# AolinFeng/PMP-VVC-TIP2023

Measured on AMD Instinct MI355X. Metric: CTUs/sec (luma QT+MTT inference+post-proc), higher is better.
Workload: dtype f16x3

## Files before the change

pmp_vvc_tip2023_amd/csrc/conv_f16x3.hip:

```cpp
#include <cstdio>
#include <type_traits>

#include "pmp_kernels.h"
#include "split3.h"

namespace pmp {

template <int KH, int KW, int NTHR = 256>
struct StagePlanH {
    unsigned off[GeoH<KH, KW, 16, NTHR>::NLD];
    unsigned valid;
};

template <int KH, int KW, int NTHR = 256>
__device__ __forceinline__ void h2_plan(StagePlanH<KH, KW, NTHR> &p, size_t plane_stride, int H, int W, int ty, int tx)
{
    typedef GeoH<KH, KW, 16, NTHR> G;
    constexpr int PY = KH / 2, PX = KW / 2;
    p.valid = 0;
#pragma unroll
    for (int k = 0; k < G::NLD; ++k) {
        const int i = min((int)threadIdx.x + k * NTHR, G::PIECES - 1);
        const int sp = i / G::PLANE, j = i - sp * G::PLANE, pix = j >> 1, half = j & 1;
        const int row = pix / G::TW, col = pix - row * G::TW;
        const int gy = ty * 16 + row - PY, gx = tx * 16 + col - PX;
        const bool in = gy >= 0 && gy < H && gx >= 0 && gx < W && (int)threadIdx.x + k * NTHR < G::PIECES;
        if (in) p.valid |= 1u << k;
        const int cy = min(max(gy, 0), H - 1), cx = min(max(gx, 0), W - 1);
        p.off[k] = (unsigned)(sp * plane_stride + ((size_t)cy * W + cx) * 16 + half * 8);
    }
}

template <int KH, int KW, int NTHR = 256>
__device__ __forceinline__ void h2_stage_load(const StagePlanH<KH, KW, NTHR> &p, const unsigned short *__restrict__ grp,
                                              u32x4 (&r)[GeoH<KH, KW, 16, NTHR>::NLD], int k0 = 0, int k1 = 1 << 20)
{
#pragma unroll
    for (int k = 0; k < GeoH<KH, KW, 16, NTHR>::NLD; ++k) {
        if (k < k0 || k >= k1) continue;
        r[k] = *reinterpret_cast<const u32x4 *>(grp + p.off[k]);
    }
}

template <int KH, int KW, int NTHR = 256>
__device__ __forceinline__ void h2_stage_store(const StagePlanH<KH, KW, NTHR> &p, u32x4 *lds, const u32x4 (&r)[GeoH<KH, KW, 16, NTHR>::NLD],
                                               int k0 = 0, int k1 = 1 << 20)
{
    typedef GeoH<KH, KW, 16, NTHR> G;
#pragma unroll
    for (int k = 0; k < G::NLD; ++k) {
        if (k < k0 || k >= k1) continue;
        const int i = min((int)threadIdx.x + k * NTHR, G::PIECES);
        const u32x4 z = {0u, 0u, 0u, 0u};
        lds[i] = ((p.valid >> k) & 1u) ? r[k] : z;
    }
}

template <int KH, int KW, int NT, bool LEAN = false>
__device__ __forceinline__ void h2_accumulate(const unsigned short *__restrict__ x, size_t plane_stride,
                                              const unsigned short *__restrict__ wpk, int C, int H, int W, int n, int ty,
                                              int tx, u32x4 *lds, f32x4 (&acc)[WaveTile<NT>::RW][WaveTile<NT>::CW])
{
    constexpr int NTHR = 256;
    typedef GeoH<KH, KW, 16, NTHR> G;
    typedef WaveTile<NT> WT;
    constexpr int RW = WT::RW, CW = WT::CW;
    const int lane = threadIdx.x & 63, wave = threadIdx.x >> 6, xl = lane & 15, g = lane >> 4;
    const int rh = wave % WT::RSPLIT, ch = wave / WT::RSPLIT;
    const int CB = C >> 4;
    const size_t grp_sz = (size_t)H * W * 16;
    const unsigned short *grp0 = x + (size_t)n * CB * grp_sz;
    constexpr bool W0DB = NT == 4;
    constexpr bool W2 = W0DB && G::TAPS == 9 && !LEAN;
    u32x4 r[G::NLD];
    StagePlanH<KH, KW, NTHR> plan;
    const bool paired = (CB & 1) == 0 && (G::TAPS & 1);
    const f16x8 *wl = reinterpret_cast<const f16x8 *>(wpk) + lane + ch * CW * 64;
    const int last = paired ? (CB / 2) * G::TAPS - 1 : CB * G::NKS - 1;
    f16x8 w0[CW], w1[CW];
    f16x8 w0n[CW];
    f16x8 w1n[CW], w0nn[CW];
    h2_plan<KH, KW, NTHR>(plan, plane_stride, H, W, ty, tx);
#pragma unroll
    for (int nt = 0; nt < CW; ++nt) {
        if (W0DB) w0n[nt] = wl[(0 * NT + nt) * 64]; else w0[nt] = wl[(0 * NT + nt) * 64];
        w1[nt] = wl[(1 * NT + nt) * 64];
        if (W2) {
            const f16x8 *w2 = wl + (size_t)min(1, last) * (2 * NT * 64);
            w0nn[nt] = w2[(0 * NT + nt) * 64]; w1n[nt] = w2[(1 * NT + nt) * 64];
        }
    }
    __syncthreads();
    h2_stage_load<KH, KW, NTHR>(plan, grp0, r);
    h2_stage_store<KH, KW, NTHR>(plan, lds, r);
    __syncthreads();
    const int pb = ((rh * RW * G::TW + xl) * 2 + (g & 1)) * 16;
    int stream = 0;
    int tapsel = g >> 1;
    constexpr int O_LAST = (((G::TAPS - 1) / KW) * G::TW + (G::TAPS - 1) % KW) * 32;
    f16x8 x0[RW], x1[RW];

    auto group = [&](auto mode_tag, auto tail_tag, int cb) {
        constexpr int MODE = decltype(mode_tag)::value;
        constexpr int TAIL = decltype(tail_tag)::value;
        constexpr bool LAST = TAIL == 2;
        constexpr int NK = MODE == 0 ? G::NKS : (MODE == 1 ? (G::TAPS - 1) / 2 : (G::TAPS - 1) / 2 + 1);
        constexpr int PER = (G::NLD + (NK > 0 ? NK : 1) - 1) / (NK > 0 ? NK : 1);
        constexpr int LAG = G::TAPS > 9 ? 3 : 2;
        constexpr bool FETCH = TAIL < 2;
        u32x4 (&rl)[G::NLD] = r;
        u32x4 (&rs)[G::NLD] = r;
        constexpr bool more = !LAST;
        const unsigned short *nxt_grp = grp0 + (size_t)min(cb + 1, CB - 1) * grp_sz;
        const int bcur = cb & 1, bprev = (cb + 1) & 1;
        const char *buf = reinterpret_cast<const char *>(lds + bcur * G::BUF);
        auto xaddr = [&](int ks) -> const char * {
            const int j = MODE == 2 ? ks - 1 : ks;
            int tA = 2 * j, tB = 2 * j + 1;
            if (MODE == 0 && tB >= G::TAPS) tB = tA;
            const int oA = ((tA / KW) * G::TW + tA % KW) * 32, oB = ((tB / KW) * G::TW + tB % KW) * 32;
            return buf + (tapsel ? oB : oA) + pb;
        };
        if constexpr (LEAN) {
            constexpr int RS = 2, SUB = RW / RS;
            const char *part = reinterpret_cast<const char *>(lds + bprev * G::BUF);
            if (NK == 0 && FETCH) h2_stage_load<KH, KW, NTHR>(plan, nxt_grp, rl);
#pragma unroll
            for (int ks = 0; ks < NK; ++ks) {
                asm volatile("" : "+v"(tapsel));
                const char *px = (MODE == 2 && ks == 0) ? (g < 2 ? part : buf) + O_LAST + pb : xaddr(ks);
                ++stream;
                const f16x8 *wf = wl + (size_t)min(stream, last) * (2 * NT * 64);
                f16x8 xa[RS], xb[RS];
                auto rd_a = [&](int h) __attribute__((always_inline)) {
#pragma unroll
                    for (int m = 0; m < RS; ++m) xa[m] = *reinterpret_cast<const f16x8 *>(px + (h * RS + m) * G::TW * 32);
                };
                auto rd_b = [&](int h) __attribute__((always_inline)) {
#pragma unroll
                    for (int m = 0; m < RS; ++m) xb[m] = *reinterpret_cast<const f16x8 *>(px + G::PLANE * 16 + (h * RS + m) * G::TW * 32);
                };
#pragma unroll
                for (int h = 0; h < SUB; ++h) {
                    rd_a(h); rd_b(h);
                    __builtin_amdgcn_sched_barrier(0);
#pragma unroll
                    for (int m = 0; m < RS; ++m)
#pragma unroll
                        for (int nt = 0; nt < CW; ++nt)
                            acc[h * RS + m][nt] = __builtin_amdgcn_mfma_f32_16x16x32_f16(w1[nt], xa[m], acc[h * RS + m][nt], 0, 0, 0);
                    __builtin_amdgcn_sched_barrier(0);
                    if (h == 0) {
#pragma unroll
                        for (int nt = 0; nt < CW; ++nt) w0[nt] = w0n[nt];
#pragma unroll
                        for (int nt = 0; nt < CW; ++nt) { w1n[nt] = wf[(1 * NT + nt) * 64]; w0n[nt] = wf[(0 * NT + nt) * 64]; }
                        if (FETCH) h2_stage_load<KH, KW, NTHR>(plan, nxt_grp, rl, ks * PER, (ks + 1) * PER);
                        if (more && ks >= LAG)
                            h2_stage_store<KH, KW, NTHR>(plan, lds + ((cb + 1) & 1) * G::BUF, rs, (ks - LAG) * PER, (ks - LAG + 1) * PER);
                    } else if (h == SUB - 1) {
#pragma unroll
                        for (int nt = 0; nt < CW; ++nt) w1[nt] = w1n[nt];
                    }
                    __builtin_amdgcn_sched_barrier(0);
#pragma unroll
                    for (int m = 0; m < RS; ++m)
#pragma unroll
                        for (int nt = 0; nt < CW; ++nt)
                            acc[h * RS + m][nt] = __builtin_amdgcn_mfma_f32_16x16x32_f16(w0[nt], xa[m], acc[h * RS + m][nt], 0, 0, 0);
                    __builtin_amdgcn_sched_barrier(0);
#pragma unroll
                    for (int m = 0; m < RS; ++m)
#pragma unroll
                        for (int nt = 0; nt < CW; ++nt)
                            acc[h * RS + m][nt] = __builtin_amdgcn_mfma_f32_16x16x32_f16(w0[nt], xb[m], acc[h * RS + m][nt], 0, 0, 0);
                    __builtin_amdgcn_sched_barrier(0);
                }
                if (MODE == 2 && ks == 0) h2_lds_barrier();
            }
        } else {
            if (NK == 0) {
                if (FETCH) h2_stage_load<KH, KW, NTHR>(plan, nxt_grp, rl);
            } else if (MODE == 2) {
                if (g >= 2) {
                    const char *pl = buf + O_LAST + pb;
#pragma unroll
                    for (int m = 0; m < RW; ++m) {
                        x0[m] = *reinterpret_cast<const f16x8 *>(pl + m * G::TW * 32);
                        x1[m] = *reinterpret_cast<const f16x8 *>(pl + G::PLANE * 16 + m * G::TW * 32);
                    }
                }
            } else {
                const char *p0x = xaddr(0);
#pragma unroll
                for (int m = 0; m < RW; ++m) x0[m] = *reinterpret_cast<const f16x8 *>(p0x + m * G::TW * 32);
            }
#pragma unroll
            for (int ks = 0; ks < NK; ++ks) {
                asm volatile("" : "+v"(tapsel));
                const char *px = (MODE == 2 && ks == 0) ? buf : xaddr(ks);
                ++stream;
                if (!(MODE == 2 && ks == 0)) {
#pragma unroll
                    for (int m = 0; m < RW; ++m) x1[m] = *reinterpret_cast<const f16x8 *>(px + G::PLANE * 16 + m * G::TW * 32);
                }
                const f16x8 *wf = wl + (size_t)min(stream, last) * (2 * NT * 64);
                __builtin_amdgcn_sched_barrier(0);
#pragma unroll
                for (int m = 0; m < RW; ++m)
#pragma unroll
                    for (int nt = 0; nt < CW; ++nt) acc[m][nt] = __builtin_amdgcn_mfma_f32_16x16x32_f16(w1[nt], x0[m], acc[m][nt], 0, 0, 0);
                __builtin_amdgcn_sched_barrier(0);
                if (W2) {
                    const f16x8 *wf2 = wl + (size_t)min(stream + 1, last) * (2 * NT * 64);
#pragma unroll
                    for (int nt = 0; nt < CW; ++nt) { w1[nt] = w1n[nt]; w0[nt] = w0n[nt]; w0n[nt] = w0nn[nt]; }
#pragma unroll
                    for (int nt = 0; nt < CW; ++nt) w1n[nt] = wf2[(1 * NT + nt) * 64];
#pragma unroll
                    for (int nt = 0; nt < CW; ++nt) w0nn[nt] = wf2[(0 * NT + nt) * 64];
                } else {
#pragma unroll
                    for (int nt = 0; nt < CW; ++nt) w1[nt] = wf[(1 * NT + nt) * 64];
                    if (W0DB) {
#pragma unroll
                        for (int nt = 0; nt < CW; ++nt) w0[nt] = w0n[nt];
#pragma unroll
                        for (int nt = 0; nt < CW; ++nt) w0n[nt] = wf[(0 * NT + nt) * 64];
                    }
                }
                if (FETCH) h2_stage_load<KH, KW, NTHR>(plan, nxt_grp, rl, ks * PER, (ks + 1) * PER);
                if (more && ks >= LAG)
                    h2_stage_store<KH, KW, NTHR>(plan, lds + ((cb + 1) & 1) * G::BUF, rs, (ks - LAG) * PER, (ks - LAG + 1) * PER);
                __builtin_amdgcn_sched_barrier(0);
#pragma unroll
                for (int m = 0; m < RW; ++m)
#pragma unroll
                    for (int nt = 0; nt < CW; ++nt) acc[m][nt] = __builtin_amdgcn_mfma_f32_16x16x32_f16(w0[nt], x0[m], acc[m][nt], 0, 0, 0);
                __builtin_amdgcn_sched_barrier(0);
                if (ks + 1 < NK) {
                    const char *pn = xaddr(ks + 1);
#pragma unroll
                    for (int m = 0; m < RW; ++m) x0[m] = *reinterpret_cast<const f16x8 *>(pn + m * G::TW * 32);
                }
                __builtin_amdgcn_sched_barrier(0);
#pragma unroll
                for (int m = 0; m < RW; ++m)
#pragma unroll
                    for (int nt = 0; nt < CW; ++nt) acc[m][nt] = __builtin_amdgcn_mfma_f32_16x16x32_f16(w0[nt], x1[m], acc[m][nt], 0, 0, 0);
                __builtin_amdgcn_sched_barrier(0);
                if (!W0DB) {
#pragma unroll
                    for (int nt = 0; nt < CW; ++nt) w0[nt] = wf[(0 * NT + nt) * 64];
                }
                __builtin_amdgcn_sched_barrier(0);
            }
            if (MODE == 1 && g < 2) {
                const char *pl = buf + O_LAST + pb;
#pragma unroll
                for (int m = 0; m < RW; ++m) {
                    x0[m] = *reinterpret_cast<const f16x8 *>(pl + m * G::TW * 32);
                    x1[m] = *reinterpret_cast<const f16x8 *>(pl + G::PLANE * 16 + m * G::TW * 32);
                }
            }
        }
        if (more) h2_stage_store<KH, KW, NTHR>(plan, lds + ((cb + 1) & 1) * G::BUF, rs, NK > LAG ? (NK - LAG) * PER : 0);
        __syncthreads();
    };

    typedef std::integral_constant<int, 0> M0;
    typedef std::integral_constant<int, 1> M1;
    typedef std::integral_constant<int, 2> M2;
    typedef std::integral_constant<int, 0> T0;
    typedef std::integral_constant<int, 1> T1;
    typedef std::integral_constant<int, 2> T2;
    if (paired) {
        for (int cb = 0; cb + 2 < CB; cb += 2) {
            group(M1{}, T0{}, cb);
            group(M2{}, T0{}, cb + 1);
        }
        group(M1{}, T1{}, CB - 2);
        group(M2{}, T2{}, CB - 1);
    } else {
        for (int cb = 0; cb + 1 < CB; ++cb) group(M0{}, T0{}, cb);
        group(M0{}, T2{}, CB - 1);
    }
}

template <int NT>
__device__ __forceinline__ void h2_epilogue(const ConvX6Args &a, f32x4 (&acc)[WaveTile<NT>::RW][WaveTile<NT>::CW], int n, int ty, int tx);

template <int NT>
__device__ __forceinline__ void h2_shortcut32(const ConvX6Args &a, int n, int ty, int tx, u32x4 *lds,
                                              f32x4 (&acc)[WaveTile<NT>::RW][WaveTile<NT>::CW])
{
    typedef WaveTile<NT> WT;
    constexpr int RW = WT::RW, CW = WT::CW;
    const int tid = threadIdx.x, lane = tid & 63, wave = tid >> 6, xl = lane & 15, g = lane >> 4;
    const int rh = wave % WT::RSPLIT, ch = wave / WT::RSPLIT;
    const int W = a.W;
    const size_t grp_sz = (size_t)a.H * W * 16;
    const unsigned short *base = a.x_sc + (size_t)n * 2 * grp_sz + ((size_t)(ty * 16) * W + tx * 16) * 16;
    __syncthreads();
    u32x4 r[8];
#pragma unroll
    for (int k = 0; k < 8; ++k) {
        const int i = tid + k * 256, grp = i >> 10, plane = (i >> 9) & 1, j = i & 511, px = j >> 1, half = j & 1;
        r[k] = *reinterpret_cast<const u32x4 *>(base + plane * a.sc_stride + grp * grp_sz + ((size_t)(px >> 4) * W + (px & 15)) * 16 + half * 8);
    }
    const f16x8 *wl = reinterpret_cast<const f16x8 *>(a.w_sc) + lane + ch * CW * 64;
    f16x8 w0[CW], w1[CW];
#pragma unroll
    for (int nt = 0; nt < CW; ++nt) { w0[nt] = wl[(0 * NT + nt) * 64]; w1[nt] = wl[(1 * NT + nt) * 64]; }
#pragma unroll
    for (int k = 0; k < 8; ++k) lds[tid + k * 256] = r[k];
    __syncthreads();
    const char *px = reinterpret_cast<const char *>(lds) + (g >> 1) * 16384 + ((rh * RW * 16 + xl) * 2 + (g & 1)) * 16;
#pragma unroll
    for (int h = 0; h < RW / 2; ++h) {
        f16x8 xa[2], xb[2];
#pragma unroll
        for (int m = 0; m < 2; ++m) {
            xa[m] = *reinterpret_cast<const f16x8 *>(px + (h * 2 + m) * 16 * 32);
            xb[m] = *reinterpret_cast<const f16x8 *>(px + 8192 + (h * 2 + m) * 16 * 32);
        }
#pragma unroll
        for (int m = 0; m < 2; ++m)
#pragma unroll
            for (int nt = 0; nt < CW; ++nt) acc[h * 2 + m][nt] = __builtin_amdgcn_mfma_f32_16x16x32_f16(w1[nt], xa[m], acc[h * 2 + m][nt], 0, 0, 0);
#pragma unroll
        for (int m = 0; m < 2; ++m)
#pragma unroll
            for (int nt = 0; nt < CW; ++nt) acc[h * 2 + m][nt] = __builtin_amdgcn_mfma_f32_16x16x32_f16(w0[nt], xa[m], acc[h * 2 + m][nt], 0, 0, 0);
#pragma unroll
        for (int m = 0; m < 2; ++m)
#pragma unroll
            for (int nt = 0; nt < CW; ++nt) acc[h * 2 + m][nt] = __builtin_amdgcn_mfma_f32_16x16x32_f16(w0[nt], xb[m], acc[h * 2 + m][nt], 0, 0, 0);
    }
}

template <int KH, int KW, int NT, int SC, bool LEAN = false>
__global__ __launch_bounds__(256, NT == 4 && !LEAN ? 2 : 3) void conv_h2_kernel(ConvX6Args a)
{
    typedef GeoH<KH, KW> G;
    __shared__ u32x4 lds[2 * G::BUF];
    const int tiles_x = a.W >> 4, tiles = tiles_x * (a.H >> 4);
    int bid = blockIdx.x;
    if ((gridDim.x & 7) == 0) bid = (bid & 7) * (gridDim.x >> 3) + (bid >> 3);
    const int n = bid / tiles, t = bid - n * tiles, ty = t / tiles_x, tx = t - ty * tiles_x;
    typedef WaveTile<NT> WT;
    constexpr int RW = WT::RW, CW = WT::CW;

    f32x4 acc[RW][CW];
#pragma unroll
    for (int m = 0; m < RW; ++m)
#pragma unroll
        for (int nt = 0; nt < CW; ++nt) acc[m][nt] = (f32x4){0.f, 0.f, 0.f, 0.f};

    h2_accumulate<KH, KW, NT, LEAN>(a.x, a.x_stride, a.w, a.Cin, a.H, a.W, n, ty, tx, lds, acc);
    if (SC == 2) h2_shortcut32<NT>(a, n, ty, tx, lds, acc);
    else if (SC) h2_accumulate<1, 1, NT, LEAN>(a.x_sc, a.sc_stride, a.w_sc, a.Csc, a.H, a.W, n, ty, tx, lds, acc);
    h2_epilogue<NT>(a, acc, n, ty, tx);
}

template <int NT>
__device__ __forceinline__ void h2_epilogue(const ConvX6Args &a, f32x4 (&acc)[WaveTile<NT>::RW][WaveTile<NT>::CW], int n, int ty, int tx)
{
    typedef WaveTile<NT> WT;
    constexpr int RW = WT::RW, CW = WT::CW;
    int tid = threadIdx.x;
    asm volatile("" : "+v"(tid));
    const int lane = tid & 63, wave = tid >> 6, xl = lane & 15, g = lane >> 4;
    const int rh = wave % WT::RSPLIT, ch = wave / WT::RSPLIT;
    const int H = a.H, W = a.W;
    const size_t grp = (size_t)H * W * 16;

    const float inv_scale = a.out_scale;
    const unsigned off0 = (unsigned)(((size_t)n * NT + ch * CW) * grp + ((size_t)(ty * 16 + rh * RW) * W + tx * 16 + xl) * 16 + g * 4);
    const unsigned row_el = (unsigned)W * 16;
    const unsigned off0w = off0 - (unsigned)(g * 4) + (unsigned)(8 * (g >> 1)) + (unsigned)(g & 1) * row_el;
    u32x4 ra[RW / 2][CW], rbv[RW / 2][CW];
    auto res_load = [&](int nt, int slot) __attribute__((always_inline)) {
#pragma unroll
        for (int m = 0; m < RW; m += 2) {
            const unsigned off = off0w + (unsigned)m * row_el + (unsigned)nt * (unsigned)grp;
            ra[m >> 1][slot] = __builtin_nontemporal_load(reinterpret_cast<const u32x4 *>(a.res + off));
            rbv[m >> 1][slot] = __builtin_nontemporal_load(reinterpret_cast<const u32x4 *>(a.res + off + a.res_stride));
        }
    };
    auto res_add = [&](int nt, int slot) __attribute__((always_inline)) {
#pragma unroll
        for (int m = 0; m < RW; m += 2) {
            u32x4 p = ra[m >> 1][slot], q = rbv[m >> 1][slot];
            rows16_swap(p);
            rows16_swap(q);
            acc[m][nt] = acc[m][nt] * inv_scale + h2_sum4_lo(p, q);
            acc[m + 1][nt] = acc[m + 1][nt] * inv_scale + h2_sum4_hi(p, q);
        }
    };
    if (a.res) {
#pragma unroll
        for (int nt = 0; nt < CW; ++nt) res_load(nt, nt);
#pragma unroll
        for (int nt = 0; nt < CW; ++nt) res_add(nt, nt);
    } else {
#pragma unroll
        for (int nt = 0; nt < CW; ++nt)
#pragma unroll
            for (int m = 0; m < RW; ++m) acc[m][nt] = acc[m][nt] * inv_scale;
    }
    float amax = 0.f;
#pragma unroll
    for (int nt = 0; nt < CW; ++nt) {
#pragma unroll
        for (int m = 0; m < RW; ++m) {
            const unsigned off = off0 + (unsigned)m * row_el + (unsigned)nt * (unsigned)grp;
            f32x4 v = acc[m][nt];
            if (a.relu) { v.x = fmaxf(v.x, 0.f); v.y = fmaxf(v.y, 0.f); v.z = fmaxf(v.z, 0.f); v.w = fmaxf(v.w, 0.f); }
            if (a.gate) v *= load_split2_4(a.gate + off, a.gate_stride);
            amax = sat_amax4(amax, v);
            acc[m][nt] = v;
        }
        if (!a.pool) {
            if (a.out_f32) {
#pragma unroll
                for (int m = 0; m < RW; ++m)
                    *reinterpret_cast<f32x4 *>(a.out_f32 + off0 + (unsigned)m * row_el + (unsigned)nt * (unsigned)grp) = acc[m][nt];
            } else {
#pragma unroll
                for (int m = 0; m < RW; m += 2) {
                    const unsigned off = off0w + (unsigned)m * row_el + (unsigned)nt * (unsigned)grp;
                    u32x4 p, q;
                    split2_rows(acc[m][nt], acc[m + 1][nt], p, q);
                    rows16_swap(p);
                    rows16_swap(q);
                    __builtin_nontemporal_store(p, reinterpret_cast<u32x4 *>(a.out + off));
                    __builtin_nontemporal_store(q, reinterpret_cast<u32x4 *>(a.out + off + a.out_stride));
                }
            }
        } else {
            const int Ho = H >> 1, Wo = W >> 1;
#pragma unroll
            for (int m = 0; m < RW; m += 2) {
                f32x4 v = acc[m][nt], u = acc[m + 1][nt];
                v.x = fmaxf(v.x, u.x); v.y = fmaxf(v.y, u.y); v.z = fmaxf(v.z, u.z); v.w = fmaxf(v.w, u.w);
                f32x4 o;
                o.x = __shfl_xor(v.x, 1); o.y = __shfl_xor(v.y, 1); o.z = __shfl_xor(v.z, 1); o.w = __shfl_xor(v.w, 1);
                v.x = fmaxf(v.x, o.x); v.y = fmaxf(v.y, o.y); v.z = fmaxf(v.z, o.z); v.w = fmaxf(v.w, o.w);
                if ((xl & 1) == 0) {
                    const int yo = ty * 8 + rh * (RW / 2) + (m >> 1), xo = tx * 8 + (xl >> 1);
                    const size_t off = (((size_t)n * NT + ch * CW + nt) * Ho + yo) * Wo * 16 + (size_t)xo * 16 + g * 4;
                    if (a.out_f32) *reinterpret_cast<f32x4 *>(a.out_f32 + off) = v;
                    else store_split2_4(a.out + off, a.out_stride, v);
                }
            }
        }
    }
    if (!a.out_f32) sat_report(a.sat, amax);
}

#define PMP_H2_LAUNCH_SC(NT, SC, LEAN)                                                                          \
    do {                                                                                                        \
        note_launch("conv_h2_kernel", KH, KW, NT, SC, LEAN);                                                    \
        hipLaunchKernelGGL((conv_h2_kernel<KH, KW, NT, SC, LEAN>), dim3(grid), dim3(256), 0, s, a);             \
    } while (0)
#define PMP_H2_LAUNCH(NT)                                                                                       \
    if (a.x_sc) PMP_H2_LAUNCH_SC(NT, 1, false);                                                                 \
    else PMP_H2_LAUNCH_SC(NT, 0, false)

template <int KH, int KW>
static hipError_t launch_h2(hipStream_t s, const ConvX6Args &a)
{
    const int grid = a.N * (a.H >> 4) * (a.W >> 4);
    switch (a.Cout >> 4) {
    case 1: PMP_H2_LAUNCH(1); break;
    case 2: PMP_H2_LAUNCH(2); break;
    case 4:
        if constexpr (KH > 1) {
            if (a.x_sc && a.Csc == 32) {
                PMP_H2_LAUNCH_SC(4, 2, false);
            } else if (!a.x_sc) {
                PMP_H2_LAUNCH_SC(4, 0, true);
            } else {
                PMP_H2_LAUNCH_SC(4, 1, false);
            }
        } else {
            PMP_H2_LAUNCH(4);
        }
        break;
    default: return hipErrorInvalidValue;
    }
    return hipGetLastError();
}
#undef PMP_H2_LAUNCH
#undef PMP_H2_LAUNCH_SC

hipError_t launch_conv_h2(hipStream_t s, const ConvX6Args &a_in)
{
    const ConvX6Args &a = a_in;

    if ((a.H & 15) || (a.W & 15) || (a.Cin & 15) || (a.Cout & 15) || (a.x_sc && (a.Csc & 15)) || a.N <= 0)
        return hipErrorInvalidValue;
// ... 45 lines not shown
```

pmp_vvc_tip2023_amd/csrc/conv_misc.hip:

```cpp
#include "pmp_kernels.h"
#include "split3.h"

namespace pmp {

__device__ __forceinline__ size_t act_idx(int n, int c, int y, int x, int CB, int H, int W)
{
    return ((((size_t)n * CB + (c >> 4)) * H + y) * W + x) * 16 + (c & 15);
}

template <int KH, int KW, int CIN, int PS, int ROWS, int FMT>
__device__ __forceinline__ void stem_conv(const float *__restrict__ planes, const float *__restrict__ w,
                                          const float *__restrict__ bias, int cout, int x, int y0, int OUT,
                                          const ActOut &out, size_t out_n, int ch_off)
{
#pragma unroll 1
    for (int c0 = 0; c0 < cout; c0 += 8) {
        float acc[ROWS][8];
#pragma unroll
        for (int r = 0; r < ROWS; ++r)
#pragma unroll
            for (int k = 0; k < 8; ++k) acc[r][k] = bias[c0 + k];
        for (int ci = 0; ci < CIN; ++ci) {
            const float *pl = planes + ci * PS * PS;
#pragma unroll
// ... 22 lines not shown
            const int c = ch_off + c0;
            const size_t o = out_n + (((size_t)(c >> 4) * OUT + (y0 + r)) * OUT + x) * 16 + (c & 15);
            f32x4 v0 = {fmaxf(acc[r][0], 0.f), fmaxf(acc[r][1], 0.f), fmaxf(acc[r][2], 0.f), fmaxf(acc[r][3], 0.f)};
            f32x4 v1 = {fmaxf(acc[r][4], 0.f), fmaxf(acc[r][5], 0.f), fmaxf(acc[r][6], 0.f), fmaxf(acc[r][7], 0.f)};
            if (FMT != FMT_F32) { out.store4(o, v0); out.store4(o + 4, v1); }
            else { *reinterpret_cast<f32x4 *>(out.f32 + o) = v0; *reinterpret_cast<f32x4 *>(out.f32 + o + 4) = v1; }
        }
    }
}

template <bool LUMA, bool MSBD, int FMT>
__global__ __launch_bounds__(256) void stem_kernel(StemArgs a)
{
    constexpr int S = LUMA ? 68 : 34, P = LUMA ? 4 : 2, PS = S + P, OUT = S - P;
    constexpr int CIN = (LUMA ? 1 : 3) + (MSBD ? 1 : 0);
    constexpr int K1 = LUMA ? 9 : 5, K2 = LUMA ? 5 : 3;
    constexpr int NW = MSBD ? (K1 * K1 * CIN * 16 + 2 * K2 * K1 * CIN * 8) : (K1 * K1 * CIN * 32);
    extern __shared__ float smem[];
    float *planes = smem;
    float *wl = smem + CIN * PS * PS;
    float *bl = wl + NW;
    const int n = blockIdx.x, tid = threadIdx.x;

    for (int i = tid; i < NW; i += 256) wl[i] = a.w[i];
    if (tid < 32) bl[tid] = a.bias[tid];
    const uint8_t *by = a.by + (size_t)n * 68 * 68;
    for (int i = tid; i < PS * PS; i += 256) {
        const int r = i / PS, c = i - r * PS;
        const bool in = r < S && c < S;
        if (LUMA) {
            planes[i] = in ? (float)by[r * 68 + c] : 0.f;
        } else {
            float v0 = 0.f, v1 = 0.f, v2 = 0.f;
            if (in) {
                const uint8_t *p = by + (2 * r) * 68 + 2 * c;
                const int m = max(max((int)p[0], (int)p[1]), max((int)p[68], (int)p[69]));
                v0 = (float)m;
                v1 = (float)a.bu[(size_t)n * 34 * 34 + r * 34 + c];
                v2 = (float)a.bv[(size_t)n * 34 * 34 + r * 34 + c];
            }
            planes[i] = v0; planes[PS * PS + i] = v1; planes[2 * PS * PS + i] = v2;
        }
        if (MSBD) {
            float qv = 0.f;
            if (in && r >= P && c >= P) {
                constexpr int SC = LUMA ? 8 : 4;
                qv = a.q[(size_t)n * 64 + ((r - P) / SC) * 8 + (c - P) / SC];
            }
            planes[(CIN - 1) * PS * PS + i] = qv;
        }
    }
    __syncthreads();

    const size_t out_n = (size_t)n * 2 * OUT * OUT * 16;
    const ActOut out{a.out, a.out_s3, a.s3_stride, FMT, a.sat};
    constexpr int COLS_PER_WG = 256 / OUT;
    constexpr int BAND = OUT / COLS_PER_WG;
    const int x = tid % OUT, band = tid / OUT;
    for (int y0 = band * BAND; y0 < (band + 1) * BAND; y0 += 4) {
        if (MSBD) {
            stem_conv<K1, K1, CIN, PS, 4, FMT>(planes, wl, bl, 16, x, y0, OUT, out, out_n, 0);
            stem_conv<K2, K1, CIN, PS, 4, FMT>(planes, wl + K1 * K1 * CIN * 16, bl + 16, 8, x, y0, OUT, out, out_n, 16);
            stem_conv<K1, K2, CIN, PS, 4, FMT>(planes, wl + K1 * K1 * CIN * 16 + K2 * K1 * CIN * 8, bl + 24, 8, x, y0, OUT,
                                          out, out_n, 24);
        } else {
            stem_conv<K1, K1, CIN, PS, 4, FMT>(planes, wl, bl, 32, x, y0, OUT, out, out_n, 0);
        }
    }
}

template <bool LUMA, bool MSBD>
__global__ __launch_bounds__(256, 2) void stem_mfma_kernel(StemArgs a)
{
    constexpr int S = LUMA ? 68 : 34, P = LUMA ? 4 : 2, PS = S + P, OUT = S - P;
    constexpr int CIN = (LUMA ? 1 : 3) + (MSBD ? 1 : 0);
    constexpr int K1 = LUMA ? 9 : 5;
    constexpr int RPS = LUMA ? 3 : 5, KPP = (K1 + RPS - 1) / RPS, KS = CIN * KPP;
    static_assert(RPS * K1 <= 32 && KPP * RPS == K1, "a K-step holds whole kernel rows, a plane whole K-steps");
    constexpr int RS = PS + 16;
    constexpr int SEGS = OUT / 16, RB = 8, NBATCH = SEGS * (OUT / RB);
    constexpr int NPIX = CIN - (MSBD ? 1 : 0);
    __shared__ _Float16 h0[NPIX * PS * RS + 16];
    __shared__ unsigned hq[MSBD ? PS * RS + 16 : 4];
    const int n = blockIdx.x, tid = threadIdx.x, lane = tid & 63, wave = tid >> 6, xl = lane & 15, g = lane >> 4;

    const uint8_t *by = a.by + (size_t)n * 68 * 68;
    for (int i = tid; i < PS * RS; i += 256) {
        const int r = i / RS, c = i - r * RS;
        const bool in = r < S && c < S;
        if (LUMA) {
            h0[i] = in ? (_Float16)(float)by[r * 68 + c] : (_Float16)0.f;
        } else {
            float v0 = 0.f, v1 = 0.f, v2 = 0.f;
            if (in) {
                const uint8_t *p = by + (2 * r) * 68 + 2 * c;
                v0 = (float)max(max((int)p[0], (int)p[1]), max((int)p[68], (int)p[69]));
                v1 = (float)a.bu[(size_t)n * 34 * 34 + r * 34 + c];
                v2 = (float)a.bv[(size_t)n * 34 * 34 + r * 34 + c];
            }
            h0[i] = (_Float16)v0; h0[PS * RS + i] = (_Float16)v1; h0[2 * PS * RS + i] = (_Float16)v2;
        }
        if (MSBD) {
            float qv = 0.f;
            if (in && r >= P && c >= P) {
                constexpr int SC = LUMA ? 8 : 4;
                qv = a.q[(size_t)n * 64 + ((r - P) / SC) * 8 + (c - P) / SC];
            }
            _Float16 q0, q1;
            sat_report(a.sat, fabsf(qv));
            split2(qv, q0, q1);
            unsigned short b0, b1;
            __builtin_memcpy(&b0, &q0, 2); __builtin_memcpy(&b1, &q1, 2);
            hq[i] = (unsigned)b0 | ((unsigned)b1 << 16);
        }
    }
    __syncthreads();

    const f16x8 *wl = reinterpret_cast<const f16x8 *>(a.wh) + lane;
    const float inv_scale = a.out_scale;
    const size_t out_n = (size_t)n * 2 * OUT * OUT * 16;
    int eo[8];
#pragma unroll
    for (int j = 0; j < 8; ++j) {
        const int kk = 8 * g + j;
        eo[j] = min(kk / K1, RPS - 1) * RS + kk % K1;
    }
    auto gather = [&](const _Float16 *p) __attribute__((always_inline)) {
        f16x8 v;
#pragma unroll
        for (int j = 0; j < 8; ++j) v[j] = p[eo[j]];
        return v;
    };
    auto gather2 = [&](const unsigned *p, f16x8 &x0v, f16x8 &x1v) __attribute__((always_inline)) {
        unsigned v[8];
#pragma unroll
        for (int j = 0; j < 8; ++j) v[j] = p[eo[j]];
        u32x4 lo, hi;
#pragma unroll
        for (int k = 0; k < 4; ++k) {
            lo[k] = __builtin_amdgcn_perm(v[2 * k + 1], v[2 * k], 0x05040100u);
            hi[k] = __builtin_amdgcn_perm(v[2 * k + 1], v[2 * k], 0x07060302u);
        }
        __builtin_memcpy(&x0v, &lo, 16);
        __builtin_memcpy(&x1v, &hi, 16);
    };
    for (int b = wave; b < NBATCH; b += 4) {
        const int seg = b % SEGS, y0 = (b / SEGS) * RB, x0 = seg * 16;
        f32x4 acc[RB][2];
        f16x8 win[RB], win1[MSBD ? RB : 1];
#pragma unroll
        for (int m = 0; m < RB; ++m) { acc[m][0] = (f32x4){0.f, 0.f, 0.f, 0.f}; acc[m][1] = (f32x4){0.f, 0.f, 0.f, 0.f}; }
        f16x8 wq[2][6];
        auto wload = [&](int ks, bool third) __attribute__((always_inline)) {
            const f16x8 *wk = wl + (size_t)ks * (3 * 2 * 64);
#pragma unroll
            for (int i = 0; i < 6; ++i)
                if (i < 4 || third) wq[ks & 1][i] = wk[i * 64];
        };
        wload(0, true);
#pragma unroll
        for (int ks = 0; ks < KS; ++ks) {
            constexpr int dummy = 0; (void)dummy;
            const int plane = ks / KPP, s = ks % KPP, r0 = s * RPS;
            const bool isq = MSBD && plane == CIN - 1;
            const _Float16 *base = h0 + ((isq ? 0 : plane) * PS + y0) * RS + x0 + xl;
            const unsigned *baseq = hq + y0 * RS + x0 + xl;
            if (s == 0) {
#pragma unroll
                for (int m = 0; m < RB; ++m) {
                    if (isq) gather2(baseq + m * RS, win[m], win1[m]);
                    else win[m] = gather(base + m * RS);
                }
            }
            __builtin_amdgcn_sched_barrier(0);
            if (ks + 1 < KS) wload(ks + 1, !(MSBD && (ks + 1) / KPP == CIN - 1));
            __builtin_amdgcn_sched_barrier(0);
            const f16x8 w00 = wq[ks & 1][0], w01 = wq[ks & 1][1], w10 = wq[ks & 1][2], w11 = wq[ks & 1][3];
#pragma unroll
            for (int m = 0; m < RB; ++m) {
                const f16x8 bx = win[(m + r0) & (RB - 1)];
                if (!isq) {
                    const f16x8 w20 = wq[ks & 1][4], w21 = wq[ks & 1][5];
                    acc[m][0] = __builtin_amdgcn_mfma_f32_16x16x32_f16(w20, bx, acc[m][0], 0, 0, 0);
                    acc[m][1] = __builtin_amdgcn_mfma_f32_16x16x32_f16(w21, bx, acc[m][1], 0, 0, 0);
                }
                acc[m][0] = __builtin_amdgcn_mfma_f32_16x16x32_f16(w10, bx, acc[m][0], 0, 0, 0);
                acc[m][1] = __builtin_amdgcn_mfma_f32_16x16x32_f16(w11, bx, acc[m][1], 0, 0, 0);
                acc[m][0] = __builtin_amdgcn_mfma_f32_16x16x32_f16(w00, bx, acc[m][0], 0, 0, 0);
                acc[m][1] = __builtin_amdgcn_mfma_f32_16x16x32_f16(w01, bx, acc[m][1], 0, 0, 0);
                if (isq) {
                    const f16x8 b1 = win1[(m + r0) & (RB - 1)];
                    acc[m][0] = __builtin_amdgcn_mfma_f32_16x16x32_f16(w00, b1, acc[m][0], 0, 0, 0);
                    acc[m][1] = __builtin_amdgcn_mfma_f32_16x16x32_f16(w01, b1, acc[m][1], 0, 0, 0);
                }
                if (s + 1 < KPP && m < RPS) {
                    const int p = RB + r0 + m;
                    if (isq) gather2(baseq + p * RS, win[p & (RB - 1)], win1[p & (RB - 1)]);
                    else win[p & (RB - 1)] = gather(base + p * RS);
                }
            }
        }
#pragma unroll
        for (int nt = 0; nt < 2; ++nt) {
            const f32x4 bias = *reinterpret_cast<const f32x4 *>(a.bias + nt * 16 + g * 4);
#pragma unroll
            for (int m = 0; m < RB; m += 2) {
                f32x4 v0 = acc[m][nt] * inv_scale + bias, v1 = acc[m + 1][nt] * inv_scale + bias;
                v0.x = fmaxf(v0.x, 0.f); v0.y = fmaxf(v0.y, 0.f); v0.z = fmaxf(v0.z, 0.f); v0.w = fmaxf(v0.w, 0.f);
                v1.x = fmaxf(v1.x, 0.f); v1.y = fmaxf(v1.y, 0.f); v1.z = fmaxf(v1.z, 0.f); v1.w = fmaxf(v1.w, 0.f);
                sat_report(a.sat, sat_amax4(sat_amax4(0.f, v0), v1));
                u32x4 p, q;
                split2_rows(v0, v1, p, q);
                rows16_swap(p);
                rows16_swap(q);
                const size_t o = out_n + (((size_t)nt * OUT + (y0 + m + (g & 1))) * OUT + x0 + xl) * 16 + 8 * (g >> 1);
                __builtin_nontemporal_store(p, reinterpret_cast<u32x4 *>(a.out_s3 + o));
                __builtin_nontemporal_store(q, reinterpret_cast<u32x4 *>(a.out_s3 + o + a.s3_stride));
            }
        }
    }
}

template <bool LUMA, bool MSBD>
static hipError_t launch_stem_t(hipStream_t s, const StemArgs &a)
{
    if (a.out_s3 && a.fmt == FMT_H2 && a.wh) {
        hipLaunchKernelGGL((stem_mfma_kernel<LUMA, MSBD>), dim3(a.N), dim3(256), 0, s, a);
        return hipGetLastError();
    }
    constexpr int S = LUMA ? 68 : 34, P = LUMA ? 4 : 2, PS = S + P;
    constexpr int CIN = (LUMA ? 1 : 3) + (MSBD ? 1 : 0);
    constexpr int K1 = LUMA ? 9 : 5, K2 = LUMA ? 5 : 3;
    constexpr int NW = MSBD ? (K1 * K1 * CIN * 16 + 2 * K2 * K1 * CIN * 8) : (K1 * K1 * CIN * 32);
    const size_t smem = (size_t)(CIN * PS * PS + NW + 32) * sizeof(float);
    if (a.out_s3 && a.fmt == FMT_H2) hipLaunchKernelGGL((stem_kernel<LUMA, MSBD, FMT_H2>), dim3(a.N), dim3(256), smem, s, a);
    else if (a.out_s3) hipLaunchKernelGGL((stem_kernel<LUMA, MSBD, FMT_B3>), dim3(a.N), dim3(256), smem, s, a);
    else hipLaunchKernelGGL((stem_kernel<LUMA, MSBD, FMT_F32>), dim3(a.N), dim3(256), smem, s, a);
    return hipGetLastError();
}

hipError_t launch_stem(hipStream_t s, bool luma, bool msbd, const StemArgs &a)
{
    if (luma) return msbd ? launch_stem_t<true, true>(s, a) : launch_stem_t<true, false>(s, a);
    return msbd ? launch_stem_t<false, true>(s, a) : launch_stem_t<false, false>(s, a);
}

__global__ __launch_bounds__(256) void conv_direct_kernel(ConvDirectArgs a)
{
    const size_t total = (size_t)a.N * a.H * a.W * a.CoutPad;
    const size_t i = (size_t)blockIdx.x * 256 + threadIdx.x;
    if (i >= total) return;
    const int co = (int)(i % a.CoutPad);
    size_t r = i / a.CoutPad;
    const int x = (int)(r % a.W); r /= a.W;
    const int y = (int)(r % a.H);
    const int n = (int)(r / a.H);
    const int CBo = a.CoutPad >> 4;
    float acc = 0.f;
    if (co < a.Cout) {
        if (a.bias) acc = a.bias[co];
        const int py = a.KH / 2, px = a.KW / 2, CBi = a.CinPad >> 4;
        for (int dy = 0; dy < a.KH; ++dy) {
            const int yy = y + dy - py;
            if (yy < 0 || yy >= a.H) continue;
            for (int dx = 0; dx < a.KW; ++dx) {
                const int xx = x + dx - px;
                if (xx < 0 || xx >= a.W) continue;
                const float *wp = a.w + (size_t)((dy * a.KW + dx) * a.Cin) * a.Cout + co;
                for (int ci = 0; ci < a.Cin; ++ci)
                    acc = fmaf(a.x[act_idx(n, ci, yy, xx, CBi, a.H, a.W)], wp[(size_t)ci * a.Cout], acc);
            }
        }
        if (a.x_sc) {
            const int CBs = a.CscPad >> 4;
            for (int ci = 0; ci < a.Csc; ++ci)
                acc = fmaf(a.x_sc[act_idx(n, ci, y, x, CBs, a.H, a.W)], a.w_sc[(size_t)ci * a.Cout + co], acc);
        }
        if (a.res) acc += a.res[act_idx(n, co, y, x, CBo, a.H, a.W)];
        if (a.relu) acc = fmaxf(acc, 0.f);
    }
    a.out[act_idx(n, co, y, x, CBo, a.H, a.W)] = acc;
}

__global__ __launch_bounds__(256) void conv_direct8_kernel(ConvDirectArgs a)
{
    extern __shared__ float wl[];
    const int taps = a.KH * a.KW, nw = taps * a.Cin;
    for (int i = threadIdx.x; i < (nw + (a.x_sc ? a.Csc : 0)) * 8; i += 256) {
        const int row = i >> 3, co = i & 7;
        float v = 0.f;
        if (co < a.Cout) v = row < nw ? a.w[(size_t)row * a.Cout + co] : a.w_sc[(size_t)(row - nw) * a.Cout + co];
        wl[i] = v;
    }
    __syncthreads();
    const size_t total = (size_t)a.N * a.H * a.W;
    const size_t i = (size_t)blockIdx.x * 256 + threadIdx.x;
    if (i >= total) return;
    const int x = (int)(i % a.W), y = (int)((i / a.W) % a.H), n = (int)(i / ((size_t)a.W * a.H));
    const int CBi = a.CinPad >> 4, CBo = a.CoutPad >> 4, py = a.KH / 2, px = a.KW / 2;
    float acc[8];
#pragma unroll
    for (int co = 0; co < 8; ++co) acc[co] = (a.bias && co < a.Cout) ? a.bias[co] : 0.f;
    auto mac16 = [&](const float *xp, const float *wp, int nch) {
        const f32x4 q0 = *reinterpret_cast<const f32x4 *>(xp), q1 = *reinterpret_cast<const f32x4 *>(xp + 4),
                    q2 = *reinterpret_cast<const f32x4 *>(xp + 8), q3 = *reinterpret_cast<const f32x4 *>(xp + 12);
        const float v[16] = {q0.x, q0.y, q0.z, q0.w, q1.x, q1.y, q1.z, q1.w, q2.x, q2.y, q2.z, q2.w, q3.x, q3.y, q3.z, q3.w};
#pragma unroll
        for (int c = 0; c < 16; ++c) {
            if (c < nch) {
                const f32x4 w0 = *reinterpret_cast<const f32x4 *>(wp + c * 8), w1 = *reinterpret_cast<const f32x4 *>(wp + c * 8 + 4);
                acc[0] = fmaf(v[c], w0.x, acc[0]); acc[1] = fmaf(v[c], w0.y, acc[1]); acc[2] = fmaf(v[c], w0.z, acc[2]); acc[3] = fmaf(v[c], w0.w, acc[3]);
                acc[4] = fmaf(v[c], w1.x, acc[4]); acc[5] = fmaf(v[c], w1.y, acc[5]); acc[6] = fmaf(v[c], w1.z, acc[6]); acc[7] = fmaf(v[c], w1.w, acc[7]);
            }
        }
    };
    for (int dy = 0; dy < a.KH; ++dy) {
        const int yy = y + dy - py;
        if (yy < 0 || yy >= a.H) continue;
        for (int dx = 0; dx < a.KW; ++dx) {
// ... 177 lines not shown
```

Before: 15380.

## Stage stem weights in LDS, batch input loads, and prefetch gate operands

The MFMA stem kernel now copies its f16 weights into shared memory once per block, so inner loops read them from LDS instead of global memory. It also hoists the bias loads and restructures the input-staging loop to issue several global loads per thread before converting and storing them. In the f16x3 conv epilogue, all gate values are loaded up front before the multiply, so their memory latency overlaps. The changes raise shared-memory and register use, which can lower occupancy, and the fallback stem path for FMT_H2 without weights now returns an error.

Measured after the change: 15520, median of 6. About the same (+0.9%).

```diff
diff --git a/pmp_vvc_tip2023_amd/csrc/conv_f16x3.hip b/pmp_vvc_tip2023_amd/csrc/conv_f16x3.hip
--- a/pmp_vvc_tip2023_amd/csrc/conv_f16x3.hip
+++ b/pmp_vvc_tip2023_amd/csrc/conv_f16x3.hip
@@ -409,15 +409,34 @@
 #pragma unroll
             for (int m = 0; m < RW; ++m) acc[m][nt] = acc[m][nt] * inv_scale;
     }
+    const bool relu_here = a.relu && !a.gate;
+    if (a.gate) {
+        u32x2_t ga[RW][CW], gb[RW][CW];
+#pragma unroll
+        for (int nt = 0; nt < CW; ++nt)
+#pragma unroll
+            for (int m = 0; m < RW; ++m) {
+                const unsigned short *gp = a.gate + off0 + (unsigned)m * row_el + (unsigned)nt * (unsigned)grp;
+                ga[m][nt] = *reinterpret_cast<const u32x2_t *>(gp);
+                gb[m][nt] = *reinterpret_cast<const u32x2_t *>(gp + a.gate_stride);
+            }
+#pragma unroll
+        for (int nt = 0; nt < CW; ++nt)
+#pragma unroll
+            for (int m = 0; m < RW; ++m) {
+                f32x4 v = acc[m][nt];
+                if (a.relu) { v.x = fmaxf(v.x, 0.f); v.y = fmaxf(v.y, 0.f); v.z = fmaxf(v.z, 0.f); v.w = fmaxf(v.w, 0.f); }
+                const u32x2_t x = ga[m][nt], y = gb[m][nt];
+                acc[m][nt] = v * (f32x4){h2_sum_lo(x.x, y.x), h2_sum_hi(x.x, y.x), h2_sum_lo(x.y, y.y), h2_sum_hi(x.y, y.y)};
+            }
+    }
     float amax = 0.f;
 #pragma unroll
     for (int nt = 0; nt < CW; ++nt) {
 #pragma unroll
         for (int m = 0; m < RW; ++m) {
-            const unsigned off = off0 + (unsigned)m * row_el + (unsigned)nt * (unsigned)grp;
             f32x4 v = acc[m][nt];
-            if (a.relu) { v.x = fmaxf(v.x, 0.f); v.y = fmaxf(v.y, 0.f); v.z = fmaxf(v.z, 0.f); v.w = fmaxf(v.w, 0.f); }
-            if (a.gate) v *= load_split2_4(a.gate + off, a.gate_stride);
+            if (relu_here) { v.x = fmaxf(v.x, 0.f); v.y = fmaxf(v.y, 0.f); v.z = fmaxf(v.z, 0.f); v.w = fmaxf(v.w, 0.f); }
             amax = sat_amax4(amax, v);
             acc[m][nt] = v;
         }
diff --git a/pmp_vvc_tip2023_amd/csrc/conv_misc.hip b/pmp_vvc_tip2023_amd/csrc/conv_misc.hip
--- a/pmp_vvc_tip2023_amd/csrc/conv_misc.hip
+++ b/pmp_vvc_tip2023_amd/csrc/conv_misc.hip
@@ -128,41 +128,66 @@
     constexpr int NPIX = CIN - (MSBD ? 1 : 0);
     __shared__ _Float16 h0[NPIX * PS * RS + 16];
     __shared__ unsigned hq[MSBD ? PS * RS + 16 : 4];
+    __shared__ f16x8 wls[KS * 3 * 2 * 64];
     const int n = blockIdx.x, tid = threadIdx.x, lane = tid & 63, wave = tid >> 6, xl = lane & 15, g = lane >> 4;
 
+    constexpr int NWF = KS * 3 * 2 * 64, WIT = (NWF + 255) / 256;
+    f16x8 wst[WIT];
+#pragma unroll
+    for (int k = 0; k < WIT; ++k) wst[k] = reinterpret_cast<const f16x8 *>(a.wh)[min(tid + k * 256, NWF - 1)];
+    const f32x4 bias0 = *reinterpret_cast<const f32x4 *>(a.bias + g * 4), bias1 = *reinterpret_cast<const f32x4 *>(a.bias + 16 + g * 4);
+
     const uint8_t *by = a.by + (size_t)n * 68 * 68;
-    for (int i = tid; i < PS * RS; i += 256) {
-        const int r = i / RS, c = i - r * RS;
-        const bool in = r < S && c < S;
-        if (LUMA) {
-            h0[i] = in ? (_Float16)(float)by[r * 68 + c] : (_Float16)0.f;
-        } else {
-            float v0 = 0.f, v1 = 0.f, v2 = 0.f;
-            if (in) {
+    constexpr int FU = LUMA ? 5 : 4;
+    for (int i0 = tid; i0 < PS * RS; i0 += 256 * FU) {
+        int pix[FU][LUMA ? 1 : 3];
+        float qv[FU];
+#pragma unroll
+        for (int k = 0; k < FU; ++k) {
+            const int i = min(i0 + k * 256, PS * RS - 1), r = min(i / RS, S - 1), c = min(i % RS, S - 1);
+            if (LUMA) {
+                pix[k][0] = by[r * 68 + c];
+            } else {
                 const uint8_t *p = by + (2 * r) * 68 + 2 * c;
-                v0 = (float)max(max((int)p[0], (int)p[1]), max((int)p[68], (int)p[69]));
-                v1 = (float)a.bu[(size_t)n * 34 * 34 + r * 34 + c];
-                v2 = (float)a.bv[(size_t)n * 34 * 34 + r * 34 + c];
-            }
-            h0[i] = (_Float16)v0; h0[PS * RS + i] = (_Float16)v1; h0[2 * PS * RS + i] = (_Float16)v2;
-        }
-        if (MSBD) {
-            float qv = 0.f;
-            if (in && r >= P && c >= P) {
+                pix[k][0] = max(max((int)p[0], (int)p[1]), max((int)p[68], (int)p[69]));
+                pix[k][1] = a.bu[(size_t)n * 34 * 34 + r * 34 + c];
+                pix[k][2] = a.bv[(size_t)n * 34 * 34 + r * 34 + c];
+            }
+            if (MSBD) {
                 constexpr int SC = LUMA ? 8 : 4;
-                qv = a.q[(size_t)n * 64 + ((r - P) / SC) * 8 + (c - P) / SC];
-            }
-            _Float16 q0, q1;
-            sat_report(a.sat, fabsf(qv));
-            split2(qv, q0, q1);
-            unsigned short b0, b1;
-            __builtin_memcpy(&b0, &q0, 2); __builtin_memcpy(&b1, &q1, 2);
-            hq[i] = (unsigned)b0 | ((unsigned)b1 << 16);
-        }
-    }
-    __syncthreads();
-
-    const f16x8 *wl = reinterpret_cast<const f16x8 *>(a.wh) + lane;
+                qv[k] = a.q[(size_t)n * 64 + ((max(r, P) - P) / SC) * 8 + (max(c, P) - P) / SC];
+            }
+        }
+#pragma unroll
+        for (int k = 0; k < FU; ++k) {
+#pragma unroll
+            for (int pl = 0; pl < (LUMA ? 1 : 3); ++pl) asm volatile("" : "+v"(pix[k][pl]));
+            if (MSBD) asm volatile("" : "+v"(qv[k]));
+        }
+#pragma unroll
+        for (int k = 0; k < FU; ++k) {
+            const int i = i0 + k * 256, r = i / RS, c = i - r * RS;
+            if (i >= PS * RS) break;
+            const bool in = r < S && c < S;
+#pragma unroll
+            for (int pl = 0; pl < (LUMA ? 1 : 3); ++pl) h0[pl * PS * RS + i] = in ? (_Float16)(float)pix[k][pl] : (_Float16)0.f;
+            if (MSBD) {
+                const float q = in && r >= P && c >= P ? qv[k] : 0.f;
+                _Float16 q0, q1;
+                sat_report(a.sat, fabsf(q));
+                split2(q, q0, q1);
+                unsigned short b0, b1;
+                __builtin_memcpy(&b0, &q0, 2); __builtin_memcpy(&b1, &q1, 2);
+                hq[i] = (unsigned)b0 | ((unsigned)b1 << 16);
+            }
+        }
+    }
+#pragma unroll
+    for (int k = 0; k < WIT; ++k)
+        if (tid + k * 256 < NWF) wls[tid + k * 256] = wst[k];
+    __syncthreads();
+
+    const f16x8 *wl = wls + lane;
     const float inv_scale = a.out_scale;
     const size_t out_n = (size_t)n * 2 * OUT * OUT * 16;
     int eo[8];
@@ -248,7 +273,7 @@
         }
 #pragma unroll
         for (int nt = 0; nt < 2; ++nt) {
-            const f32x4 bias = *reinterpret_cast<const f32x4 *>(a.bias + nt * 16 + g * 4);
+            const f32x4 bias = nt ? bias1 : bias0;
 #pragma unroll
             for (int m = 0; m < RB; m += 2) {
                 f32x4 v0 = acc[m][nt] * inv_scale + bias, v1 = acc[m + 1][nt] * inv_scale + bias;
@@ -270,7 +295,8 @@
 template <bool LUMA, bool MSBD>
 static hipError_t launch_stem_t(hipStream_t s, const StemArgs &a)
 {
-    if (a.out_s3 && a.fmt == FMT_H2 && a.wh) {
+    if (a.out_s3 && a.fmt == FMT_H2) {
+        if (!a.wh) return hipErrorInvalidValue;
         hipLaunchKernelGGL((stem_mfma_kernel<LUMA, MSBD>), dim3(a.N), dim3(256), 0, s, a);
         return hipGetLastError();
     }
@@ -279,8 +305,7 @@
     constexpr int K1 = LUMA ? 9 : 5, K2 = LUMA ? 5 : 3;
     constexpr int NW = MSBD ? (K1 * K1 * CIN * 16 + 2 * K2 * K1 * CIN * 8) : (K1 * K1 * CIN * 32);
     const size_t smem = (size_t)(CIN * PS * PS + NW + 32) * sizeof(float);
-    if (a.out_s3 && a.fmt == FMT_H2) hipLaunchKernelGGL((stem_kernel<LUMA, MSBD, FMT_H2>), dim3(a.N), dim3(256), smem, s, a);
-    else if (a.out_s3) hipLaunchKernelGGL((stem_kernel<LUMA, MSBD, FMT_B3>), dim3(a.N), dim3(256), smem, s, a);
+    if (a.out_s3) hipLaunchKernelGGL((stem_kernel<LUMA, MSBD, FMT_B3>), dim3(a.N), dim3(256), smem, s, a);
     else hipLaunchKernelGGL((stem_kernel<LUMA, MSBD, FMT_F32>), dim3(a.N), dim3(256), smem, s, a);
     return hipGetLastError();
 }
```

## Use lean low-register path for 5x5 NT=4 shortcut convs to raise occupancy

Applied to the files above, without the earlier changes.

For 5x5 kernels with NT=4 and a shortcut, the kernel now takes the LEAN accumulation form and its launch bounds target 3 waves per SIMD instead of 2. To fit the tighter register budget it adds a SLIM mode: branchless tap-address selection through a mask, opaque asm barriers on offsets and thread ids to stop the compiler hoisting or duplicating address math, and a new generic 1x1 shortcut routine that steps through channel groups. Higher occupancy should hide more latency, at the risk of register spills or weaker software pipelining in the shortcut path.

Measured after the change: 15650 before, 15810 after, median of 6. +1.0%, better.

```diff
diff --git a/pmp_vvc_tip2023_amd/csrc/conv_f16x3.hip b/pmp_vvc_tip2023_amd/csrc/conv_f16x3.hip
--- a/pmp_vvc_tip2023_amd/csrc/conv_f16x3.hip
+++ b/pmp_vvc_tip2023_amd/csrc/conv_f16x3.hip
@@ -31,18 +31,20 @@
     }
 }
 
-template <int KH, int KW, int NTHR = 256>
+template <int KH, int KW, int NTHR = 256, bool OPQ = false>
 __device__ __forceinline__ void h2_stage_load(const StagePlanH<KH, KW, NTHR> &p, const unsigned short *__restrict__ grp,
                                               u32x4 (&r)[GeoH<KH, KW, 16, NTHR>::NLD], int k0 = 0, int k1 = 1 << 20)
 {
 #pragma unroll
     for (int k = 0; k < GeoH<KH, KW, 16, NTHR>::NLD; ++k) {
         if (k < k0 || k >= k1) continue;
-        r[k] = *reinterpret_cast<const u32x4 *>(grp + p.off[k]);
-    }
-}
-
-template <int KH, int KW, int NTHR = 256>
+        unsigned off = p.off[k];
+        if (OPQ) asm volatile("" : "+v"(off));
+        r[k] = *reinterpret_cast<const u32x4 *>(grp + off);
+    }
+}
+
+template <int KH, int KW, int NTHR = 256, bool OPQ = false>
 __device__ __forceinline__ void h2_stage_store(const StagePlanH<KH, KW, NTHR> &p, u32x4 *lds, const u32x4 (&r)[GeoH<KH, KW, 16, NTHR>::NLD],
                                                int k0 = 0, int k1 = 1 << 20)
 {
@@ -50,13 +52,15 @@
 #pragma unroll
     for (int k = 0; k < G::NLD; ++k) {
         if (k < k0 || k >= k1) continue;
-        const int i = min((int)threadIdx.x + k * NTHR, G::PIECES);
+        int tid = threadIdx.x;
+        if (OPQ) asm volatile("" : "+v"(tid));
+        const int i = min(tid + k * NTHR, G::PIECES);
         const u32x4 z = {0u, 0u, 0u, 0u};
         lds[i] = ((p.valid >> k) & 1u) ? r[k] : z;
     }
 }
 
-template <int KH, int KW, int NT, bool LEAN = false>
+template <int KH, int KW, int NT, bool LEAN = false, bool SLIM = false>
 __device__ __forceinline__ void h2_accumulate(const unsigned short *__restrict__ x, size_t plane_stride,
                                               const unsigned short *__restrict__ wpk, int C, int H, int W, int n, int ty,
                                               int tx, u32x4 *lds, f32x4 (&acc)[WaveTile<NT>::RW][WaveTile<NT>::CW])
@@ -96,7 +100,7 @@
     __syncthreads();
     const int pb = ((rh * RW * G::TW + xl) * 2 + (g & 1)) * 16;
     int stream = 0;
-    int tapsel = g >> 1;
+    int tapsel = SLIM ? -(g >> 1) : g >> 1;
     constexpr int O_LAST = (((G::TAPS - 1) / KW) * G::TW + (G::TAPS - 1) % KW) * 32;
     f16x8 x0[RW], x1[RW];
 
@@ -119,6 +123,7 @@
             int tA = 2 * j, tB = 2 * j + 1;
             if (MODE == 0 && tB >= G::TAPS) tB = tA;
             const int oA = ((tA / KW) * G::TW + tA % KW) * 32, oB = ((tB / KW) * G::TW + tB % KW) * 32;
+            if (SLIM) return buf + (oA + pb) + (tapsel & (oB - oA));
             return buf + (tapsel ? oB : oA) + pb;
         };
         if constexpr (LEAN) {
@@ -155,9 +160,9 @@
                         for (int nt = 0; nt < CW; ++nt) w0[nt] = w0n[nt];
 #pragma unroll
                         for (int nt = 0; nt < CW; ++nt) { w1n[nt] = wf[(1 * NT + nt) * 64]; w0n[nt] = wf[(0 * NT + nt) * 64]; }
-                        if (FETCH) h2_stage_load<KH, KW, NTHR>(plan, nxt_grp, rl, ks * PER, (ks + 1) * PER);
+                        if (FETCH) h2_stage_load<KH, KW, NTHR, SLIM>(plan, nxt_grp, rl, ks * PER, (ks + 1) * PER);
                         if (more && ks >= LAG)
-                            h2_stage_store<KH, KW, NTHR>(plan, lds + ((cb + 1) & 1) * G::BUF, rs, (ks - LAG) * PER, (ks - LAG + 1) * PER);
+                            h2_stage_store<KH, KW, NTHR, SLIM>(plan, lds + ((cb + 1) & 1) * G::BUF, rs, (ks - LAG) * PER, (ks - LAG + 1) * PER);
                     } else if (h == SUB - 1) {
 #pragma unroll
                         for (int nt = 0; nt < CW; ++nt) w1[nt] = w1n[nt];
@@ -290,13 +295,15 @@
 template <int NT>
 __device__ __forceinline__ void h2_epilogue(const ConvX6Args &a, f32x4 (&acc)[WaveTile<NT>::RW][WaveTile<NT>::CW], int n, int ty, int tx);
 
-template <int NT>
+template <int NT, bool OPQ = false>
 __device__ __forceinline__ void h2_shortcut32(const ConvX6Args &a, int n, int ty, int tx, u32x4 *lds,
                                               f32x4 (&acc)[WaveTile<NT>::RW][WaveTile<NT>::CW])
 {
     typedef WaveTile<NT> WT;
     constexpr int RW = WT::RW, CW = WT::CW;
-    const int tid = threadIdx.x, lane = tid & 63, wave = tid >> 6, xl = lane & 15, g = lane >> 4;
+    int tid = threadIdx.x;
+    if (OPQ) asm volatile("" : "+v"(tid));
+    const int lane = tid & 63, wave = tid >> 6, xl = lane & 15, g = lane >> 4;
     const int rh = wave % WT::RSPLIT, ch = wave / WT::RSPLIT;
     const int W = a.W;
     const size_t grp_sz = (size_t)a.H * W * 16;
@@ -339,8 +346,65 @@
     }
 }
 
+template <int NT>
+__device__ __forceinline__ void h2_shortcut_any(const ConvX6Args &a, int n, int ty, int tx, u32x4 *lds,
+                                                f32x4 (&acc)[WaveTile<NT>::RW][WaveTile<NT>::CW])
+{
+    typedef WaveTile<NT> WT;
+    constexpr int RW = WT::RW, CW = WT::CW;
+    int tid = threadIdx.x;
+    asm volatile("" : "+v"(tid));
+    const int lane = tid & 63, wave = tid >> 6, xl = lane & 15, g = lane >> 4;
+    const int rh = wave % WT::RSPLIT, ch = wave / WT::RSPLIT;
+    const int W = a.W;
+    const size_t grp_sz = (size_t)a.H * W * 16;
+    const int CB = a.Csc >> 4, per = (CB & 1) ? 1 : 2, steps = CB / per;
+    const unsigned short *base = a.x_sc + (size_t)n * CB * grp_sz + ((size_t)(ty * 16) * W + tx * 16) * 16;
+    for (int s = 0; s < steps; ++s) {
+        __syncthreads();
+        u32x4 r[8];
+#pragma unroll
+        for (int k = 0; k < 8; ++k) {
+            const int i = tid + k * 256, grp = s * per + (per == 2 ? i >> 10 : 0), plane = (i >> 9) & 1, j = i & 511, pix = j >> 1, half = j & 1;
+            r[k] = *reinterpret_cast<const u32x4 *>(base + plane * a.sc_stride + grp * grp_sz + ((size_t)(pix >> 4) * W + (pix & 15)) * 16 + half * 8);
+        }
+        const f16x8 *wf = reinterpret_cast<const f16x8 *>(a.w_sc) + lane + ch * CW * 64 + (size_t)s * (2 * NT * 64);
+        f16x8 w0[CW], w1[CW];
+#pragma unroll
+        for (int nt = 0; nt < CW; ++nt) { w0[nt] = wf[(0 * NT + nt) * 64]; w1[nt] = wf[(1 * NT + nt) * 64]; }
+#pragma unroll
+        for (int k = 0; k < 8; ++k) lds[tid + k * 256] = r[k];
+        __syncthreads();
+        const char *px = reinterpret_cast<const char *>(lds) + (g >> 1) * 16384 + ((rh * RW * 16 + xl) * 2 + (g & 1)) * 16;
+#pragma unroll
+        for (int h = 0; h < RW / 2; ++h) {
+            f16x8 xa[2], xb[2];
+#pragma unroll
+            for (int m = 0; m < 2; ++m) {
+                xa[m] = *reinterpret_cast<const f16x8 *>(px + (h * 2 + m) * 16 * 32);
+                xb[m] = *reinterpret_cast<const f16x8 *>(px + 8192 + (h * 2 + m) * 16 * 32);
+            }
+#pragma unroll
+            for (int m = 0; m < 2; ++m)
+#pragma unroll
+                for (int nt = 0; nt < CW; ++nt) acc[h * 2 + m][nt] = __builtin_amdgcn_mfma_f32_16x16x32_f16(w1[nt], xa[m], acc[h * 2 + m][nt], 0, 0, 0);
+#pragma unroll
+            for (int m = 0; m < 2; ++m)
+#pragma unroll
+                for (int nt = 0; nt < CW; ++nt) acc[h * 2 + m][nt] = __builtin_amdgcn_mfma_f32_16x16x32_f16(w0[nt], xa[m], acc[h * 2 + m][nt], 0, 0, 0);
+#pragma unroll
+            for (int m = 0; m < 2; ++m)
+#pragma unroll
+                for (int nt = 0; nt < CW; ++nt) acc[h * 2 + m][nt] = __builtin_amdgcn_mfma_f32_16x16x32_f16(w0[nt], xb[m], acc[h * 2 + m][nt], 0, 0, 0);
+        }
+    }
+}
+
+template <int KH, int NT, int SC, bool LEAN>
+constexpr bool h2_lean_form = LEAN || (KH == 5 && NT == 4 && SC != 0);
+
 template <int KH, int KW, int NT, int SC, bool LEAN = false>
-__global__ __launch_bounds__(256, NT == 4 && !LEAN ? 2 : 3) void conv_h2_kernel(ConvX6Args a)
+__global__ __launch_bounds__(256, (NT == 4 && !h2_lean_form<KH, NT, SC, LEAN> ? 2 : 3)) void conv_h2_kernel(ConvX6Args a)
 {
     typedef GeoH<KH, KW> G;
     __shared__ u32x4 lds[2 * G::BUF];
@@ -357,9 +421,12 @@
 #pragma unroll
         for (int nt = 0; nt < CW; ++nt) acc[m][nt] = (f32x4){0.f, 0.f, 0.f, 0.f};
 
-    h2_accumulate<KH, KW, NT, LEAN>(a.x, a.x_stride, a.w, a.Cin, a.H, a.W, n, ty, tx, lds, acc);
-    if (SC == 2) h2_shortcut32<NT>(a, n, ty, tx, lds, acc);
-    else if (SC) h2_accumulate<1, 1, NT, LEAN>(a.x_sc, a.sc_stride, a.w_sc, a.Csc, a.H, a.W, n, ty, tx, lds, acc);
+    constexpr bool LF = h2_lean_form<KH, NT, SC, LEAN>;
+    constexpr bool SLIM = LF && KH == 5;
+    h2_accumulate<KH, KW, NT, LF, SLIM>(a.x, a.x_stride, a.w, a.Cin, a.H, a.W, n, ty, tx, lds, acc);
+    if (SC == 2) h2_shortcut32<NT, SLIM>(a, n, ty, tx, lds, acc);
+    else if (SC && SLIM) h2_shortcut_any<NT>(a, n, ty, tx, lds, acc);
+    else if (SC) h2_accumulate<1, 1, NT, LF, SLIM>(a.x_sc, a.sc_stride, a.w_sc, a.Csc, a.H, a.W, n, ty, tx, lds, acc);
     h2_epilogue<NT>(a, acc, n, ty, tx);
 }
 
```
